# cmgcds/SParSH-AMG

Hardware: AMD Instinct MI355X
Metric: AMG-PCG solve iterations/sec (7-pt 3D Poisson, fp64) + HBM GB/s (roofline: dominant kernel; config.whole_iteration: the iteration) (higher is better)
Workload: dtype f64

## Files before the change

include/sparsh_amg.h:

```cpp
#ifndef SPARSH_AMG_H_
#define SPARSH_AMG_H_

#ifdef __cplusplus
extern "C" {
#endif

#define SPARSH_OK 0
#define SPARSH_EINVAL -1
#define SPARSH_ENODEV -2
#define SPARSH_ESTATE -3
#define SPARSH_ENUMERIC -4
#define SPARSH_ENOCONV -5
#define SPARSH_ECOMM -6

#define SPARSH_AMG 0
#define SPARSH_CG 1
#define SPARSH_PCG 2
#define SPARSH_BICG 3
#define SPARSH_PBICG 4
#define SPARSH_GMRES 5
#define SPARSH_PGMRES 6
#define SPARSH_FCG 7
#define SPARSH_BCG 8
#define SPARSH_MBICG 10
// ... 26 lines not shown
    int extend_until;
    int coarse_factor_mb;
} sparsh_params;

typedef struct sparsh_handle_s *sparsh_handle;

const char *sparsh_last_error(void);
int sparsh_version(void);
int sparsh_device_count(void);
int sparsh_host_cpus(void);

void sparsh_default_params(sparsh_params *p);

int sparsh_create_csr(int nrow, int ncol, const int *rowptr, const int *colindex, const double *val, sparsh_handle *out);
void sparsh_destroy(sparsh_handle h);

int sparsh_setup(sparsh_handle h, const sparsh_params *p);

int sparsh_set_stopping(sparsh_handle h, double tol, int max_iter, int check_every);

int sparsh_set_kernel_config(sparsh_handle h, int kind, int vec, int nt, int remap);

int sparsh_level_format(sparsh_handle h, int level, int *kind, long *stored_entries);

int sparsh_level_layout(sparsh_handle h, int level, long *slots, long *value_blocks, long *meta_bytes);
int sparsh_set_const_slots(sparsh_handle h, int enable);
int sparsh_set_index_compression(sparsh_handle h, int mode);
int sparsh_set_alternate_sweeps(sparsh_handle h, int mode);
int sparsh_set_paired_restriction(sparsh_handle h, int enable);
int sparsh_set_fused_prolongation(sparsh_handle h, int enable);
int sparsh_set_constant_diagonal(sparsh_handle h, int enable);
int sparsh_set_double_sweep(sparsh_handle h, int mode);
int sparsh_set_marching_ops(sparsh_handle h, int mode);
int sparsh_set_zero_start(sparsh_handle h, int enable);
int sparsh_set_deferred_x(sparsh_handle h, int enable);
int sparsh_level_marching_ops(sparsh_handle h, int level, int *on, int *plan, double *table_us, double *marching_us);
int sparsh_set_box_plan(sparsh_handle h, int level, int kernel, int q, int ty, int cz);
int sparsh_set_box_plan_ex(sparsh_handle h, int level, int kernel, int threads, int q, int ty, int cz);
int sparsh_level_box_threads(sparsh_handle h, int level, int *double_threads, int *marching_threads);
int sparsh_debug_box_plan_candidates(int kernel, int nx, int ny, int nz, int part_cap, int cap, int *plans);
int sparsh_level_double_sweep(sparsh_handle h, int level, int *on, int *dims, int *plan, double *single_us, double *double_us);
int sparsh_level_constant_diagonal(sparsh_handle h, int level, int *is_const, double *value);
int sparsh_level_prolong_fused(sparsh_handle h, int level, int *fused);
int sparsh_level_paired(sparsh_handle h, int level, int *paired);
int sparsh_set_fused_zero_sweep(sparsh_handle h, int mode);
int sparsh_set_placement_search(sparsh_handle h, int enable);
int sparsh_placement_info(sparsh_handle h, double *chosen_us, double *worst_us, double *initial_us, int *triples, double *seconds);
int sparsh_set_setup_broadcast(sparsh_handle h, int enable);
int sparsh_setup_share_info(sparsh_handle h, int *built_locally, long *image_bytes);
long sparsh_debug_hierarchy_roundtrip(sparsh_handle h, long truncate_to);
int sparsh_level_index16(sparsh_handle h, int level, long *blocks16, long *blocks);
int sparsh_debug_index16_roundtrip(int nrow, const int *rowptr, const int *colindex, long *blocks16, long *blocks);
int sparsh_set_tile(sparsh_handle h, int enable);
int sparsh_level_tile_rows(sparsh_handle h, int level, int *rows);
int sparsh_bench_comm(sparsh_handle h, int what, int level, int reps, double *avg_seconds);
const char *sparsh_level_kernel(sparsh_handle h, int level);
int sparsh_level_placement(sparsh_handle h, int level, int *nt, int *remap);

int sparsh_setup_host(sparsh_handle h, const sparsh_params *p);

int sparsh_num_levels(sparsh_handle h);
int sparsh_level_info(sparsh_handle h, int level, int *nrow, int *nnz, int *p_ncol, int *p_nnz);
int sparsh_level_csr(sparsh_handle h, int level, int which, int *rowptr, int *colindex, double *val);
int sparsh_coarse_inverse(sparsh_handle h, double *inv);
int sparsh_coarse_info(sparsh_handle h, int *info6, long *bytes);
int sparsh_set_coarse_form(sparsh_handle h, int form, int leaf, int merge_rows);
// ... 233 lines not shown
```

sparsh_amg_amd/__init__.py:

```python
from __future__ import annotations

import ctypes as C
import os

import numpy as np

from . import problems

_HERE = os.path.dirname(os.path.abspath(__file__))
LIB_PATH = os.path.join(_HERE, "libsparsh_amg.so")

SPARSH_AMG, SPARSH_CG, SPARSH_PCG, SPARSH_BICG, SPARSH_PBICG = 0, 1, 2, 3, 4
SPARSH_GMRES, SPARSH_PGMRES = 5, 6
SPARSH_FCG = 7
METHODS = {"amg": SPARSH_AMG, "cg": SPARSH_CG, "pcg": SPARSH_PCG, "bicg": SPARSH_BICG, "pbicg": SPARSH_PBICG,
           "gmres": SPARSH_GMRES, "pgmres": SPARSH_PGMRES}
SPARSH_BCG = 8
BLOCK_METHODS = {"bcg": SPARSH_BCG}
SPARSH_MBICG = 10
UNSYMMETRIC_BLOCK_METHODS = {"mbicg": SPARSH_MBICG}
SPARSH_MBICG_SCALARS, SPARSH_MBICG_PARTIALS = 9, 2048
MBICG_SLOTS = ("ALPHA1", "APR0", "ALPHA", "ASS", "ASAS", "OMEGA1", "BETA", "RR0", "RES")
MBICG_FIN = {"init": 0, "alpha": 1, "omega": 2, "beta_res": 3}
FLEXIBLE_METHODS = {"fcg": SPARSH_FCG}
# ... 63 lines not shown

def _load():
    if not os.path.exists(LIB_PATH):
        raise ImportError(
            f"{LIB_PATH} is missing: build it with `python -c 'import __graft_entry__ as g; g.build()'` "
            "(or `make -C sparsh_amg_amd/csrc`).  There is no pure-Python/CPU fallback."
        )
    L = C.CDLL(LIB_PATH)
    H = C.c_void_p
    P = C.POINTER
    sig = {
        "sparsh_last_error": (C.c_char_p, []),
        "sparsh_version": (C.c_int, []),
        "sparsh_device_count": (C.c_int, []),
        "sparsh_host_cpus": (C.c_int, []),
        "sparsh_default_params": (None, [P(Params)]),
        "sparsh_create_csr": (C.c_int, [C.c_int, C.c_int, c_int_p, c_int_p, c_dbl_p, P(H)]),
        "sparsh_destroy": (None, [H]),
        "sparsh_setup": (C.c_int, [H, P(Params)]),
        "sparsh_setup_host": (C.c_int, [H, P(Params)]),
        "sparsh_set_stopping": (C.c_int, [H, C.c_double, C.c_int, C.c_int]),
        "sparsh_set_kernel_config": (C.c_int, [H, C.c_int, C.c_int, C.c_int, C.c_int]),
        "sparsh_level_placement": (C.c_int, [H, C.c_int, c_int_p, c_int_p]),
        "sparsh_level_format": (C.c_int, [H, C.c_int, c_int_p, C.POINTER(C.c_long)]),
        "sparsh_level_layout": (C.c_int, [H, C.c_int, C.POINTER(C.c_long), C.POINTER(C.c_long), C.POINTER(C.c_long)]),
        "sparsh_set_const_slots": (C.c_int, [H, C.c_int]),
        "sparsh_set_tile": (C.c_int, [H, C.c_int]),
        "sparsh_set_index_compression": (C.c_int, [H, C.c_int]),
        "sparsh_set_alternate_sweeps": (C.c_int, [H, C.c_int]),
        "sparsh_set_paired_restriction": (C.c_int, [H, C.c_int]),
        "sparsh_set_fused_prolongation": (C.c_int, [H, C.c_int]),
        "sparsh_set_constant_diagonal": (C.c_int, [H, C.c_int]),
        "sparsh_set_double_sweep": (C.c_int, [H, C.c_int]),
        "sparsh_set_marching_ops": (C.c_int, [H, C.c_int]),
        "sparsh_set_zero_start": (C.c_int, [H, C.c_int]),
        "sparsh_set_deferred_x": (C.c_int, [H, C.c_int]),
        "sparsh_level_marching_ops": (C.c_int, [H, C.c_int, C.POINTER(C.c_int), C.POINTER(C.c_int), C.POINTER(C.c_double), C.POINTER(C.c_double)]),
        "sparsh_level_double_sweep": (C.c_int, [H, C.c_int, C.POINTER(C.c_int), C.POINTER(C.c_int), C.POINTER(C.c_int), C.POINTER(C.c_double),
                                                  C.POINTER(C.c_double)]),
        "sparsh_level_constant_diagonal": (C.c_int, [H, C.c_int, C.POINTER(C.c_int), C.POINTER(C.c_double)]),
        "sparsh_level_prolong_fused": (C.c_int, [H, C.c_int, C.POINTER(C.c_int)]),
        "sparsh_op_jacobi_prolong": (C.c_int, [H, C.c_int, c_dbl_p, c_dbl_p, c_dbl_p]),
        "sparsh_set_box_plan": (C.c_int, [H, C.c_int, C.c_int, C.c_int, C.c_int, C.c_int]),
        "sparsh_set_box_plan_ex": (C.c_int, [H, C.c_int, C.c_int, C.c_int, C.c_int, C.c_int, C.c_int]),
        "sparsh_level_box_threads": (C.c_int, [H, C.c_int, c_int_p, c_int_p]),
        "sparsh_debug_box_plan_candidates": (C.c_int, [C.c_int, C.c_int, C.c_int, C.c_int, C.c_int, C.c_int, c_int_p]),
        "sparsh_op_spmv_dot": (C.c_int, [H, C.c_int, c_dbl_p, c_dbl_p, c_dbl_p]),
        "sparsh_op_jacobi_dot": (C.c_int, [H, C.c_int, c_dbl_p, c_dbl_p, c_dbl_p, c_dbl_p]),
        "sparsh_level_paired": (C.c_int, [H, C.c_int, C.POINTER(C.c_int)]),
        "sparsh_set_fused_zero_sweep": (C.c_int, [H, C.c_int]),
        "sparsh_set_placement_search": (C.c_int, [H, C.c_int]),
        "sparsh_placement_info": (C.c_int, [H, C.POINTER(C.c_double), C.POINTER(C.c_double), C.POINTER(C.c_double), c_int_p, C.POINTER(C.c_double)]),
        "sparsh_debug_index16_roundtrip": (C.c_int, [C.c_int, c_int_p, c_int_p, C.POINTER(C.c_long), C.POINTER(C.c_long)]),
        "sparsh_set_setup_broadcast": (C.c_int, [H, C.c_int]),
        "sparsh_debug_hierarchy_roundtrip": (C.c_long, [H, C.c_long]),
        "sparsh_setup_share_info": (C.c_int, [H, C.POINTER(C.c_int), C.POINTER(C.c_long)]),
        "sparsh_level_index16": (C.c_int, [H, C.c_int, C.POINTER(C.c_long), C.POINTER(C.c_long)]),
        "sparsh_level_tile_rows": (C.c_int, [H, C.c_int, c_int_p]),
        "sparsh_bench_comm": (C.c_int, [H, C.c_int, C.c_int, C.c_int, c_dbl_p]),
        "sparsh_level_kernel": (C.c_char_p, [H, C.c_int]),
        "sparsh_num_levels": (C.c_int, [H]),
        "sparsh_level_info": (C.c_int, [H, C.c_int, c_int_p, c_int_p, c_int_p, c_int_p]),
        "sparsh_level_csr": (C.c_int, [H, C.c_int, C.c_int, c_int_p, c_int_p, c_dbl_p]),
        "sparsh_coarse_inverse": (C.c_int, [H, c_dbl_p]),
        "sparsh_op_precond_f32": (C.c_int, [H, c_dbl_p, c_dbl_p]),
        "sparsh_level_f32_layout": (C.c_int, [H, C.c_int, c_int_p]),
# ... 354 lines not shown
    def hierarchy_roundtrip(self, truncate_to=-1):
        r = lib.sparsh_debug_hierarchy_roundtrip(self._h, int(truncate_to))
        if r < 0:
            _check(int(r))
        return int(r)

    def setup_share_info(self):
        a, b = C.c_int(), C.c_long()
        _check(lib.sparsh_setup_share_info(self._h, C.byref(a), C.byref(b)))
        return bool(a.value), b.value

    def set_placement_search(self, enable=True):
        _check(lib.sparsh_set_placement_search(self._h, int(bool(enable))))
        return self

    def placement_info(self):
        a, b, c, k, t = C.c_double(), C.c_double(), C.c_double(), C.c_int(), C.c_double()
        _check(lib.sparsh_placement_info(self._h, C.byref(a), C.byref(b), C.byref(c), C.byref(k), C.byref(t)))
        return {"chosen_us": round(a.value, 2), "worst_us": round(b.value, 2), "initial_us": round(c.value, 2), "triples": k.value,
                "seconds": round(t.value, 3)}

    def set_fused_zero_sweep(self, enable=2):
        _check(lib.sparsh_set_fused_zero_sweep(self._h, int(enable)))
        return self

    def set_alternate_sweeps(self, mode=1):
        _check(lib.sparsh_set_alternate_sweeps(self._h, int(mode)))
        return self

    def set_double_sweep(self, mode=1):
        _check(lib.sparsh_set_double_sweep(self._h, int(mode)))
        return self

    def level_double_sweep(self, level):
        on = C.c_int(0)
        dims, plan = (C.c_int * 3)(), (C.c_int * 3)()
        t1, t2 = C.c_double(0.0), C.c_double(0.0)
        _check(lib.sparsh_level_double_sweep(self._h, int(level), C.byref(on), dims, plan, C.byref(t1), C.byref(t2)))
        return {"on": bool(on.value), "grid": list(dims), "points_per_thread": plan[0], "lines_per_tile": plan[1], "planes_per_chunk": plan[2],
                "two_single_sweeps_us": round(t1.value, 2), "double_sweep_us": round(t2.value, 2)}

    def set_deferred_x(self, enable=True):
        _check(lib.sparsh_set_deferred_x(self._h, 1 if enable else 0))
        return self

    def set_zero_start(self, enable=True):
        _check(lib.sparsh_set_zero_start(self._h, 1 if enable else 0))
        return self

    def set_marching_ops(self, mode=1):
        _check(lib.sparsh_set_marching_ops(self._h, int(mode)))
        return self

    def level_marching_ops(self, level):
        on = C.c_int(0)
        plan = (C.c_int * 3)()
        t1, t2 = C.c_double(0.0), C.c_double(0.0)
        _check(lib.sparsh_level_marching_ops(self._h, int(level), C.byref(on), plan, C.byref(t1), C.byref(t2)))
        return {"on": bool(on.value), "points_per_thread": plan[0], "lines_per_tile": plan[1], "planes_per_chunk": plan[2],
                "table_kernel_us": round(t1.value, 2), "marching_kernel_us": round(t2.value, 2)}

    def set_box_plan(self, level, kernel, q=0, ty=0, cz=0, shared_cu=False, threads=1024):
        k = {"double": 2, "marching": 1}.get(kernel, kernel)
        if shared_cu:
            if k != 1:
                raise ValueError("shared_cu is a plan of the marching kernel")
# ... 1209 lines not shown
```

sparsh_amg_amd/csrc/capi.cpp:

```cpp
#include <algorithm>
#include <cmath>
#include <cstdio>
#include <cstdlib>
#include <cstring>
#include <memory>
#include <string>
#include <vector>

#include <hip/hip_runtime_api.h>

#include "../../include/sparsh_amg.h"
#include "bcg_small.hpp"
#include "eig_chol.hpp"
#include "eig_small.hpp"
#include "engine.hpp"

using namespace sparsh;

struct sparsh_handle_s {
    std::unique_ptr<Engine> eng;
    LocalOp cached_op;
    DeepLocal cached_deep;
};

// ... 364 lines not shown
    if (!h || !h->eng) return fail(SPARSH_EINVAL, "null handle");
    if (chosen_us) *chosen_us = h->eng->place_best_us;
    if (worst_us) *worst_us = h->eng->place_worst_us;
    if (initial_us) *initial_us = h->eng->place_first_us;
    if (triples) *triples = h->eng->place_tried;
    if (seconds) *seconds = h->eng->place_seconds;
    return SPARSH_OK;
}

int sparsh_set_fused_zero_sweep(sparsh_handle h, int enable)
{
    if (!h || !h->eng) return fail(SPARSH_EINVAL, "null handle");
    h->eng->kernel_cfg().fuse_cg_zero = enable != 0;
    h->eng->kernel_cfg().cg_nt = enable == 2;
    h->eng->config_changed();
    return SPARSH_OK;
}

int sparsh_set_alternate_sweeps(sparsh_handle h, int enable)
{
    if (!h || !h->eng) return fail(SPARSH_EINVAL, "null handle");
    if (enable < 0 || enable > 2) return fail(SPARSH_EINVAL, "mode must be 0 (never), 1 (where a sweep streams more than the Infinity Cache holds) or 2 (always)");
    h->eng->kernel_cfg().alt_dir = enable;
    h->eng->config_changed();
    return SPARSH_OK;
}

int sparsh_set_double_sweep(sparsh_handle h, int mode)
{
    if (!h || !h->eng) return fail(SPARSH_EINVAL, "null handle");
    if (mode < 0 || mode > 2) return fail(SPARSH_EINVAL, "mode must be 0 (never), 1 (where the setup measures it faster) or 2 (wherever the level is a box grid with a plan)");
    h->eng->kernel_cfg().box2 = mode;
    h->eng->config_changed();
    return SPARSH_OK;
}

int sparsh_level_double_sweep(sparsh_handle h, int level, int *on, int *dims, int *plan, double *single_us, double *double_us)
{
    REQUIRE_READY(h);
    REQUIRE_LEVEL(h, level);
    const DevLevel &L = h->eng->level(level);
    if (on) *on = (!h->eng->distributed() || L.replicated) && box2_applies(L.A, h->eng->kernel_cfg()) ? 1 : 0;
    if (dims) {
        dims[0] = L.A.box_nx;
        dims[1] = L.A.box_ny;
        dims[2] = L.A.box_nz;
    }
    if (plan) {
        plan[0] = L.A.box2.q;
        plan[1] = L.A.box2.ty;
        plan[2] = L.A.box2.cz;
    }
    if (single_us) *single_us = L.box_single_us;
    if (double_us) *double_us = L.box_double_us;
    return SPARSH_OK;
}

int sparsh_set_deferred_x(sparsh_handle h, int enable)
{
    if (!h || !h->eng) return fail(SPARSH_EINVAL, "null handle");
    h->eng->kernel_cfg().defer_x = enable != 0;
    h->eng->config_changed();
    return SPARSH_OK;
}

int sparsh_set_zero_start(sparsh_handle h, int enable)
// ... 2994 lines not shown
```

sparsh_amg_amd/csrc/engine.cpp:

```cpp
#include "engine.hpp"

#include <algorithm>
#include <functional>
#include <cmath>
#include <cstdio>
#include <cstdlib>
#include <cstring>
#include <omp.h>

namespace sparsh {

namespace {
constexpr int kProfEvents = 8192;
}

bool Engine::check(hipError_t e, const char *what)
{
    if (e == hipSuccess) return true;
    error = std::string(what) + ": " + hipGetErrorString(e);
    return false;
}

bool Engine::note_hip(hipError_t e, const char *what)
{
// ... 625 lines not shown
    }
    for (size_t off = 0; good && off < total; off += chunk) {
        const size_t nb = std::min(chunk, total - off);
        if (me == 0) good = check(hipMemcpyAsync(stage, image.data() + off, nb, hipMemcpyHostToDevice, st_), "hipMemcpy");
        good = good && comm_->bcast(stage, nb, 0, st_);
        if (good && me != 0) good = check(hipMemcpyAsync(image.data() + off, stage, nb, hipMemcpyDeviceToHost, st_), "hipMemcpy");
        good = good && check(hipStreamSynchronize(st_), "hipStreamSynchronize");
    }
    if (stage) (void)hipFree(stage);
    if (!good) {
        if (error.empty()) error = "broadcast of the hierarchy failed: " + comm_->error;
        return SPARSH_ECOMM;
    }
    if (me != 0) {
        prm_ = p;
        ready_ = false;
        if (!deserialize_hierarchy(image.data(), image.size(), A0_, H_)) {
            error = H_.error;
            host_ready_ = false;
            return SPARSH_ENUMERIC;
        }
        host_ready_ = true;
        setup_seconds = omp_get_wtime() - t0;
        H_.seconds = setup_seconds;
    }
    return SPARSH_OK;
}

void Engine::tune_box_kernels()
{
    for (size_t l = 0; l + 1 < lev_.size(); ++l) {
        DevLevel &L = lev_[l];
        L.A.box_on = L.A.box1_on = false;
        L.box_single_us = L.box_double_us = L.box1_table_us = L.box1_us = 0.0;
        if (L.A.box2.q <= 0 || (dist_ && !L.replicated) || L.deep || csr_family(L.A, cfg_) != FAM_SDIA_TAB) continue;
        if (cfg_.box2 >= 2) L.A.box_on = true;
        if (cfg_.box1 >= 2) L.A.box1_on = L.A.box1.q > 0;
        const bool time2 = cfg_.box2 == 1, time1 = cfg_.box1 == 1 && L.A.box1.q > 0;
        if (!(time1 || time2)) continue;
        if (L.n < 60000) continue;
        hipEvent_t e0 = nullptr, e1 = nullptr;
        if (hipEventCreate(&e0) != hipSuccess || hipEventCreate(&e1) != hipSuccess) continue;
        CsrArgs a;
        a.b = L.r;
        launch_fill(L.n, 1.0, L.r, st_);
        a.d = L.diag;
        a.omega = prm_.omega;
        auto timed = [&](bool fused) -> double {
            double *p = L.x, *q = L.x2;
            const int launches = fused ? 5 : 10;
            for (int it = 0; it < launches; ++it) {
                if (it == (fused ? 1 : 2)) (void)hipEventRecord(e0, st_);
                if (fused) {
                    launch_box2(L.A, p, a.b, q, prm_.omega, L.fine, st_);
                } else {
                    a.x = p;
                    a.y = q;
                    launch_csr(L.A, OP_JACOBI, a, L.fine, st_, cfg_);
                }
                std::swap(p, q);
            }
            (void)hipEventRecord(e1, st_);
            if (hipEventSynchronize(e1) != hipSuccess) return 1e30;
            float ms = 0.f;
            (void)hipEventElapsedTime(&ms, e0, e1);
            return (double)ms * 1e3 / 4.0;
// ... 2008 lines not shown
```

sparsh_amg_amd/csrc/engine.hpp:

```cpp
#pragma once

#include <memory>
#include <string>
#include <vector>

#include "../../include/sparsh_amg.h"
#include "cheby_bounds.hpp"
#include "coarse.hpp"
#include "comm.hpp"
#include "dist.hpp"
#include "host_setup.hpp"
#include "kernels.hpp"

namespace sparsh {

struct DevLevel {
    bool deep = false;
    int K = 0;
    int npad = 0;
    std::vector<int> layer_end;
    DevDeepPlan dplan[3];
    std::vector<int> blk_first, wblk_first;
    double *xc_stage = nullptr;
    double *b_ext = nullptr;
// ... 116 lines not shown
    static constexpr int kCycleDefaultStride = 3;
    static constexpr long kCycleMaxVisits = 1024;
    void set_cycle(int kind, int stride)
    {
        cycle_kind_ = kind;
        cycle_stride_ = stride;
        config_changed();
    }
    int cycle_kind() const { return cycle_kind_; }
    int cycle_stride() const { return cycle_stride_; }
    bool wk_level(int l) const { return wk_level_for(l, cycle_stride_); }
    long level_visits(int l) const { return level_visits_for(l, cycle_stride_); }
    long cycle_visits() const { return cycle_visits_for(cycle_stride_); }
    int wk_level_count() const;
    size_t wk_bytes() const { return wk_bytes_; }
    void set_nullspace(int kind) { ns_kind_ = kind; }
    int nullspace_built() const { return host_ready_ ? H_.nullspace : SPARSH_NULLSPACE_NONE; }
    bool ns_on() const { return nullspace_built() == SPARSH_NULLSPACE_CONSTANT; }
    int pinned_row() const { return host_ready_ ? H_.pinned_row : -1; }
    double row_defect() const { return host_ready_ ? ns_row_defect_ : 0.0; }
    double col_defect() const { return host_ready_ ? ns_col_defect_ : 0.0; }
    void project(double *v, const double *r = nullptr, double *dot_partial = nullptr, int *dot_nblk = nullptr);
    void project_any(int n, double *v, const double *r, double *part, double *dot_partial, int *dot_nblk);
    int op_project(int n, double *v, const double *r, double *mean, double *dot);
    int cycle_check(int method);
    int cycle_prepare(int method);
    int op_kstep(int l, const double *b, const double *c, const double *d, double *r, double *x, double *scal8);
    int smoother_prepare();
    static constexpr int kSorDefaultSweeps = 6;
    static constexpr long kSorSingleNnz = 0;
    KernelConfig &kernel_cfg() { return cfg_; }
    const KernelConfig &kernel_cfg() const { return cfg_; }
    void config_changed() { drop_graph(); }
    const double *diag_stream(const DevLevel &L) const { return cfg_.const_diag && L.diag_is_const ? nullptr : L.diag; }
    bool zero_start(const DevLevel &L) const { return cfg_.zero_start && (!dist_ || L.replicated) && !L.deep && box2_applies(L.A, cfg_); }
    bool level_prolong_fused(int l) const
    {
        if (l < 1 || l + 1 >= (int)lev_.size() || !cfg_.fuse_prolong || prm_.sweeps < 1 || prm_.precond_fp32) return false;
        const DevLevel &F = lev_[l - 1];
        if (dist_ && !F.replicated) return false;
        return F.P_is_aggregation && !F.deep && (F.pair_aggregates || F.members) && F.R.nrow == lev_[l].n;
    }
    int level_paired(int l) const
    {
        if (!(l + 2 < (int)lev_.size() && prm_.sweeps > 0 && (!dist_ || lev_[l].replicated) && cfg_.pair_restrict)) return 0;
        if (lev_[l].pair_aggregates && resid_pair_applies(lev_[l].A, cfg_)) return 1;
        if (lev_[l].pair_axis != 0 && lev_[l].A.box_nx > 0 && csr_family(lev_[l].A, cfg_) == FAM_SDIA_TAB) return 1 + std::abs(lev_[l].pair_axis);
        return 0;
    }
    double bench_comm(int what, int level, int reps);
    hipStream_t stream() const { return st_; }
    double *partials() const { return part0_; }
    const DevLevel &level(int l) const { return lev_[l]; }
    int n0() const { return A0_.nrow; }
    int local_n0() const { return lev_.empty() ? A0_.nrow : lev_[0].n; }
    void set_comm(std::unique_ptr<Comm> c) { comm_ = std::move(c); }
    void set_overlap(bool on) { overlap_ = on; }
    void set_deep_halo(bool on) { deep_halo_ = on; }
    bool deep_halo() const { return deep_halo_; }
    void set_comm_tuning(int mode) { comm_tune_ = mode; }
    struct CommLevelChoice {
        int rows = 0, halo_rows = 0;
        bool partitioned = false, deep = false;
        double cost_deep_us = 0.0, cost_per_sweep_us = 0.0, cost_replicated_us = 0.0;
    };
    struct CommMeasured {
// ... 397 lines not shown
```

sparsh_amg_amd/csrc/kernels.hip:

```cpp
#include <hip/hip_runtime.h>

#include "kernels.hpp"

#include <algorithm>
#include <type_traits>
#include <vector>

namespace sparsh {

namespace {


__device__ __forceinline__ double wave_sum(double v)
{
#pragma unroll
    for (int off = 32; off > 0; off >>= 1) v += __shfl_down(v, off, 64);
    return v;
}

__device__ __forceinline__ double block_sum(double v, double *red)
{
    v = wave_sum(v);
    const int lane = threadIdx.x & 63, w = threadIdx.x >> 6;
    if (lane == 0) red[w] = v;
    __syncthreads();
    double s = 0.0;
    if (threadIdx.x == 0) {
#pragma unroll
        for (int k = 0; k < kBlock / 64; ++k) s += red[k];
    }
    return s;
}

__device__ __forceinline__ int xcd_remap(int b, int nblk, int mode)
{
// ... 1118 lines not shown

constexpr int kDivWindow = 256;
constexpr unsigned kDivWindowWidth = (unsigned)(2 * kDivWindow + 1) << 20;
struct DivConst {
    double b, r0;
    unsigned fast;
};
__device__ __forceinline__ unsigned div_window_pos(double v)
{
    return ((unsigned)__double2hiint(v) & 0x7fffffffu) - ((unsigned)(1023 - kDivWindow) << 20);
}
__device__ __forceinline__ DivConst make_div_const(double b)
{
    DivConst c;
    c.b = b;
    bool f;
    const double bs0 = __builtin_amdgcn_div_scale(1.0, b, false, &f);
    double r = __builtin_amdgcn_rcp(bs0);
    double e = __builtin_fma(-bs0, r, 1.0);
    r = __builtin_fma(r, e, r);
    e = __builtin_fma(-bs0, r, 1.0);
    r = __builtin_fma(r, e, r);
    c.r0 = r;
    c.fast = div_window_pos(b) < kDivWindowWidth && bs0 == b ? kDivWindowWidth : 0u;
    return c;
}
__device__ __forceinline__ double div_const(double a, const DivConst &c)
{
    if (__builtin_expect(__builtin_amdgcn_ballot_w64(div_window_pos(a) >= c.fast) != 0ull, 0)) return a / c.b;
    const double q0 = a * c.r0;
    const double rem = __builtin_fma(-c.b, q0, a);
    return __builtin_fma(rem, c.r0, q0);
}

struct BoxArgs {
    int nx, ny, nz;
    int TY, CZ, ytiles;
    double c[7];
    double omega;
};

template <int BS, int Q, int TAG, bool ZERO>
__global__ __launch_bounds__(BS) void sdia_box2_kernel(BoxArgs g, const double *__restrict__ x, const double *__restrict__ b,
                                                        double *__restrict__ y)
{
    extern __shared__ double box_lds[];
    const int nx = g.nx, ny = g.ny, nz = g.nz, P = nx * ny, TY = g.TY;
    const int R0 = (TY + 4) * nx;
    const int pitch = nx + 1;
    const int cells = (TY + 4) * pitch + 1;
    double *X0 = box_lds;
    double *X1 = box_lds + cells;
    int wg = blockIdx.x;
    {
        const int nwg = gridDim.x, per = nwg / 8, rem = nwg % 8;
        const int c = wg % 8, r = wg / 8;
        wg = c * per + min(c, rem) + r;
    }
    const int tile = wg % g.ytiles, zc = wg / g.ytiles;
    const int j0 = tile * TY;
    const int z0 = zc * g.CZ, z1 = min(z0 + g.CZ, nz);
    const long base = (long)(j0 - 2) * nx;
    const int tid = threadIdx.x;
    const double c0 = g.c[0], c1 = g.c[1], c2 = g.c[2], c3 = g.c[3], c4 = g.c[4], c5 = g.c[5], c6 = g.c[6], om = g.omega;
    const DivConst dc = make_div_const(c3);
    for (int i = tid; i < 2 * cells; i += BS) box_lds[i] = 0.0;
// ... 87 lines not shown
                    double sum = 0.0;
                    sum = sum + c0 * x1m[q];
                    sum = sum + c1 * X1[s - pitch];
                    sum = sum + c2 * X1[s - 1];
                    sum = sum + c3 * x1c[q];
                    sum = sum + c4 * X1[s + 1];
                    sum = sum + c5 * X1[s + pitch];
                    sum = sum + c6 * x1k[q];
                    const double h = 1.0 * bp[q] + (-1.0) * sum;
                    y[(long)k2 * P + base + p] = x1c[q] + div_const(om * h, dc);
                }
            }
        }
        __syncthreads();
#pragma unroll
        for (int q = 0; q < Q; ++q) {
            if (v1[q]) X1[sidx[q]] = x1k[q];
            x1m[q] = x1c[q];
            x1c[q] = x1k[q];
            xm[q] = xc[q];
            xc[q] = xp[q];
            bp[q] = bk[q];
            if constexpr (ZERO) {
                bk[q] = bq[q];
                bq[q] = xn[q];
                xp[q] = 0.0;
                if (v0[q] && k + 1 <= z1 && k + 2 < nz) xp[q] = div_const(om * xn[q], dc);
            } else {
                xp[q] = xn[q];
                bk[q] = bn[q];
            }
        }
    }
}

enum BoxEpi : int { BOX_SPMV_DOT = 0, BOX_JACOBI_DOT = 1, BOX_RESID_PAIRX = 2, BOX_JACOBI_PROLONG = 3, BOX_JACOBI = 4 };

struct Box1Args {
    const double *x, *b;
    double *y;
    double *y2;
    const double *dc;
    double dconst;
    const int *members;
    int nfine;
    double *partial;
};

template <int BS, int Q, int EPI, int TAG>
__global__ __launch_bounds__(BS) void sdia_box1_kernel(BoxArgs g, Box1Args a)
{
    extern __shared__ double box_lds[];
    __shared__ double red[BS / 64];
    const int nx = g.nx, ny = g.ny, nz = g.nz, P = nx * ny, TY = g.TY;
    const int R0 = (TY + 2) * nx;
    const int pitch = nx + 1;
    const int cells = (TY + 2) * pitch + 1;
    double *X0 = box_lds;
    int wg = blockIdx.x;
    {
        const int nwg = gridDim.x, per = nwg / 8, rem = nwg % 8;
        const int c = wg % 8, r = wg / 8;
        wg = c * per + min(c, rem) + r;
    }
    const int tile = wg % g.ytiles, zc = wg / g.ytiles;
    const int j0 = tile * TY;
// ... 100 lines not shown
                const double rn = lane_from_above(ri, 0.0);
                if (v1[q] && !(tid & 1)) {
                    const long J = row >> 1;
                    double bc = 0.0 + ri;
                    bc = bc + rn;
                    a.y[J] = bc;
                    if (a.y2) a.y2[J] = om * bc / (a.dc ? a.dc[J] : a.dconst);
                }
            }
        }
        __syncthreads();
#pragma unroll
        for (int q = 0; q < Q; ++q) {
            xm[q] = xc[q];
            xc[q] = xp[q];
            xp[q] = xn[q];
            bk[q] = bn[q];
        }
    }
    if constexpr (EPI == BOX_SPMV_DOT || EPI == BOX_JACOBI_DOT) {
        acc = wave_sum(acc);
        const int lane = tid & 63, w = tid >> 6;
        if (lane == 0) red[w] = acc;
        __syncthreads();
        if (tid == 0) {
            double t = 0.0;
#pragma unroll
            for (int q = 0; q < BS / 64; ++q) t += red[q];
            a.partial[blockIdx.x] = t;
        }
    }
}

__device__ __forceinline__ double box_residual(const BoxArgs &g, const double *__restrict__ x, const double *__restrict__ b, int f, int i, int j,
                                               int k)
{
    const int nx = g.nx, P = g.nx * g.ny;
    const double xm2 = k > 0 ? x[f - P] : 0.0;
    const double xm1 = j > 0 ? x[f - nx] : 0.0;
    const double xm0 = i > 0 ? x[f - 1] : 0.0;
    const double xc = x[f];
    const double xp0 = i < nx - 1 ? x[f + 1] : 0.0;
    const double xp1 = j < g.ny - 1 ? x[f + nx] : 0.0;
    const double xp2 = k < g.nz - 1 ? x[f + P] : 0.0;
    const double bi = b[f];
    double sum = 0.0;
    sum = sum + g.c[0] * xm2;
    sum = sum + g.c[1] * xm1;
    sum = sum + g.c[2] * xm0;
    sum = sum + g.c[3] * xc;
    sum = sum + g.c[4] * xp0;
    sum = sum + g.c[5] * xp1;
    sum = sum + g.c[6] * xp2;
    return 1.0 * bi + (-1.0) * sum;
}

template <int AXIS>
__global__ __launch_bounds__(kBlock) void box_resid_pair_kernel(BoxArgs g, int nc, int rev, const double *__restrict__ x, const double *__restrict__ b,
                                                                const double *__restrict__ dc, double dconst, double *__restrict__ bc,
                                                                double *__restrict__ xc)
{
    const int J = blockIdx.x * kBlock + threadIdx.x;
    if (J >= nc) return;
    const int nx = g.nx, ny = g.ny;
    const int cny = AXIS == 1 ? ny / 2 : ny;
    const int i = J % nx, t = J / nx;
// ... 250 lines not shown
}

namespace {

BoxArgs box_args(const DevCsr &A, double omega, const BoxPlan &p = {})
{
    BoxArgs g;
    g.nx = A.box_nx;
    g.ny = A.box_ny;
    g.nz = A.box_nz;
    g.TY = p.ty;
    g.CZ = p.cz;
    g.ytiles = p.ty > 0 ? (g.ny + p.ty - 1) / p.ty : 0;
    for (int u = 0; u < 7; ++u) g.c[u] = A.sd_tab.cval[u];
    g.omega = omega;
    return g;
}

template <class F>
void box_dispatch(const BoxPlan &p, F &&f)
{
    auto with_q = [&](auto bs) {
        if (p.q == 4) f(bs, std::integral_constant<int, 4>{});
        else if (p.q == 3) f(bs, std::integral_constant<int, 3>{});
        else f(bs, std::integral_constant<int, 2>{});
    };
    if (p.threads == 256) with_q(std::integral_constant<int, 256>{});
    else if (p.threads == 512) with_q(std::integral_constant<int, 512>{});
    else with_q(std::integral_constant<int, 1024>{});
}

}

bool box1_applies(const DevCsr &A, const KernelConfig &c)
{
    return c.box1 != 0 && A.box1_on && A.box1.q > 0 && csr_family(A, c) == FAM_SDIA_TAB;
}

int launch_box1(const DevCsr &A, int epi, const CsrArgs &a, bool finest, hipStream_t st)
{
    const BoxArgs g = box_args(A, a.omega, A.box1);
    Box1Args b;
    b.x = a.x;
    b.b = a.b;
    b.y = a.y;
    b.y2 = a.y2;
    b.dc = a.d;
    b.dconst = a.dconst;
    b.members = a.members;
    b.nfine = a.nfine;
    b.partial = a.partial ? a.partial + a.partial_off : nullptr;
    const int nwg = A.box1.workgroups(g.ny, g.nz);
    const dim3 grid(nwg), block(A.box1.threads);
    const size_t lds = box_lds_bytes(1, g.nx, g.TY);
    auto launch = [&](auto e) {
        box_dispatch(A.box1, [&](auto bs, auto q) {
            constexpr int BS = decltype(bs)::value, Q = decltype(q)::value, E = decltype(e)::value;
            if (finest) hipLaunchKernelGGL((sdia_box1_kernel<BS, Q, E, 1>), grid, block, lds, st, g, b);
            else hipLaunchKernelGGL((sdia_box1_kernel<BS, Q, E, 0>), grid, block, lds, st, g, b);
        });
    };
    switch (epi) {
    case BOX_SPMV_DOT: launch(std::integral_constant<int, BOX_SPMV_DOT>{}); break;
    case BOX_JACOBI_DOT: launch(std::integral_constant<int, BOX_JACOBI_DOT>{}); break;
    case BOX_RESID_PAIRX: launch(std::integral_constant<int, BOX_RESID_PAIRX>{}); break;
    case BOX_JACOBI: launch(std::integral_constant<int, BOX_JACOBI>{}); break;
    default: launch(std::integral_constant<int, BOX_JACOBI_PROLONG>{}); break;
    }
    return nwg;
}

bool box2_applies(const DevCsr &A, const KernelConfig &c)
{
    return c.box2 != 0 && A.box_on && A.box2.q > 0 && csr_family(A, c) == FAM_SDIA_TAB;
}

void launch_box2(const DevCsr &A, const double *x, const double *b, double *y, double omega, bool finest, hipStream_t st, bool from_zero)
{
    const BoxArgs g = box_args(A, omega, A.box2);
    const dim3 grid(A.box2.workgroups(g.ny, g.nz)), block(A.box2.threads);
    const size_t lds = box_lds_bytes(2, g.nx, g.TY);
    box_dispatch(A.box2, [&](auto bs, auto q) {
        constexpr int BS = decltype(bs)::value, Q = decltype(q)::value;
        if (from_zero) {
            if (finest) hipLaunchKernelGGL((sdia_box2_kernel<BS, Q, 1, true>), grid, block, lds, st, g, x, b, y);
            else hipLaunchKernelGGL((sdia_box2_kernel<BS, Q, 0, true>), grid, block, lds, st, g, x, b, y);
        } else {
            if (finest) hipLaunchKernelGGL((sdia_box2_kernel<BS, Q, 1, false>), grid, block, lds, st, g, x, b, y);
            else hipLaunchKernelGGL((sdia_box2_kernel<BS, Q, 0, false>), grid, block, lds, st, g, x, b, y);
        }
    });
}

void launch_box_resid_pair(const DevCsr &A, int axis, const double *x, const double *b, const double *dc, double dconst, double omega,
                           double *bc, double *xc, hipStream_t st)
{
    const BoxArgs g = box_args(A, omega);
    const int nc = A.nrow / 2;
    if (nc <= 0) return;
    const dim3 grid((nc + kBlock - 1) / kBlock), block(kBlock);
    const int rev = axis < 0 ? 1 : 0;
    if (axis == 1 || axis == -1)
        hipLaunchKernelGGL(box_resid_pair_kernel<1>, grid, block, 0, st, g, nc, rev, x, b, dc, dconst, bc, xc);
    else
        hipLaunchKernelGGL(box_resid_pair_kernel<2>, grid, block, 0, st, g, nc, rev, x, b, dc, dconst, bc, xc);
}

bool resid_pair_applies(const DevCsr &A, const KernelConfig &c)
{
    return c.pair_restrict && csr_family(A, c) == FAM_SDIA_TAB && sdia_tile_rows(A, c) == 0 && A.nslice > 0;
}

void launch_resid_pair(const DevCsr &A, const CsrArgs &a, bool finest, hipStream_t st, const KernelConfig &c)
{
    bool nt;
    int remap;
// ... 903 lines not shown
```

sparsh_amg_amd/csrc/kernels.hpp:

```cpp
#pragma once

#include <hip/hip_runtime_api.h>

#include <vector>

#include "box_plan.hpp"

namespace sparsh {

struct SdTable {
    int nd = 0;
    int near = 0;
    int off[8] = {0, 0, 0, 0, 0, 0, 0, 0};
    double cval[8] = {0, 0, 0, 0, 0, 0, 0, 0};
};

struct DevCsr {
    int nrow = 0, ncol = 0, nnz = 0;
    int *rowptr = nullptr;
    int *col = nullptr;
    double *val = nullptr;
    int *rowblk = nullptr;
    int nblk = 0;
    unsigned short *col16 = nullptr;
    int *cbase = nullptr;
    int nblk16 = 0;
    int *waveblk = nullptr;
    int nwblk = 0;
    int nslice = 0;
    int *slice_ptr = nullptr;
    int *sell_col = nullptr;
    double *sell_val = nullptr;
    long sell_entries = 0;
    int *sd_ptr = nullptr;
    int *sd_off = nullptr;
    unsigned long long *sd_mask = nullptr;
    double *sd_val = nullptr;
    long sd_slots = 0;
    int *sd_vidx = nullptr;
    double *sd_cval = nullptr;
    long sd_vblocks = 0;
    int *sd_rec = nullptr;
    SdTable sd_tab;
    unsigned long long *sd_tmask = nullptr;
    int *sd_tconf = nullptr;
    bool has_sdia() const { return sd_ptr != nullptr; }
    int box_nx = 0, box_ny = 0, box_nz = 0;
    BoxPlan box2;
    bool box_on = false;
    BoxPlan box1;
    bool box1_on = false;
    int *int_list = nullptr, *bnd_list = nullptr;
    int nint = 0, nbnd = 0;
};

struct KernelConfig {
    int kind = 3;
    int vec = 3;
    bool auto_policy = true;
    bool nt = true;
    int remap = 1;
    bool table = true;
    bool tile = false;
    bool const_slots = true;
    bool place_search = true;
    bool cg_nt = true;
    bool fuse_cg_zero = true;
    int alt_dir = 1;
    bool defer_x = true;
    bool zero_start = true;
    int box1 = 1;
    int box2 = 1;
    bool const_diag = true;
    bool fuse_prolong = true;
    bool pair_restrict = true;
    int idx16 = 1;
};

enum CsrFamily : int { FAM_CSR_BLOCK = 0, FAM_CSR_WAVE = 1, FAM_SELL = 2, FAM_SDIA = 3, FAM_SDIA_TAB = 4, FAM_CSR_ROWLANE = 5, FAM_CSR_ROWLANE16 = 6 };

constexpr int kBlock = 256;
constexpr int kEwGridMax = 2048;
constexpr int kStreamNnz = 2048;
constexpr int kWaveNnz = 512;
constexpr int kSdRecInts = 48;
constexpr int kSdConstBit = 1 << 30;
constexpr int kSdPlainBit = 1 << 29;
constexpr int kSdPtrMask = (1 << 29) - 1;
constexpr int kCsrPad = 4;

enum CsrOp : int {
    OP_SPMV = 0,
    OP_RESID = 1,
    OP_JACOBI = 2,
    OP_ADD = 3,
    OP_SPMV_DOT = 4,
    OP_RESNORM = 5,
    OP_JACOBI_DOT = 6,
    OP_JACOBI_PROLONG = 8,
    OP_CHEBY = 9,
    OP_CHEBY_DOT = 10,
    OP_RESID_PAIR = 7
};

struct CsrArgs {
// ... 281 lines not shown
```

Before: 711.4.

## Add branch-free box stencil kernels using clamped buffer loads and masked stores

```diff
diff --git a/include/sparsh_amg.h b/include/sparsh_amg.h
--- a/include/sparsh_amg.h
+++ b/include/sparsh_amg.h
@@ -82,6 +82,7 @@
 int sparsh_set_constant_diagonal(sparsh_handle h, int enable);
 int sparsh_set_double_sweep(sparsh_handle h, int mode);
 int sparsh_set_marching_ops(sparsh_handle h, int mode);
+int sparsh_set_box_step(sparsh_handle h, int step);
 int sparsh_set_zero_start(sparsh_handle h, int enable);
 int sparsh_set_deferred_x(sparsh_handle h, int enable);
 int sparsh_level_marching_ops(sparsh_handle h, int level, int *on, int *plan, double *table_us, double *marching_us);
diff --git a/sparsh_amg_amd/__init__.py b/sparsh_amg_amd/__init__.py
--- a/sparsh_amg_amd/__init__.py
+++ b/sparsh_amg_amd/__init__.py
@@ -119,6 +119,7 @@
         "sparsh_set_fused_prolongation": (C.c_int, [H, C.c_int]),
         "sparsh_set_constant_diagonal": (C.c_int, [H, C.c_int]),
         "sparsh_set_double_sweep": (C.c_int, [H, C.c_int]),
+        "sparsh_set_box_step": (C.c_int, [H, C.c_int]),
         "sparsh_set_marching_ops": (C.c_int, [H, C.c_int]),
         "sparsh_set_zero_start": (C.c_int, [H, C.c_int]),
         "sparsh_set_deferred_x": (C.c_int, [H, C.c_int]),
@@ -539,6 +540,10 @@
         _check(lib.sparsh_set_double_sweep(self._h, int(mode)))
         return self
 
+    def set_box_step(self, step=1):
+        _check(lib.sparsh_set_box_step(self._h, int(step)))
+        return self
+
     def level_double_sweep(self, level):
         on = C.c_int(0)
         dims, plan = (C.c_int * 3)(), (C.c_int * 3)()
diff --git a/sparsh_amg_amd/csrc/box_step.hpp b/sparsh_amg_amd/csrc/box_step.hpp
--- /dev/null
+++ b/sparsh_amg_amd/csrc/box_step.hpp
@@ -0,0 +1,33 @@
+#pragma once
+
+#if defined(__HIPCC__)
+#define SPARSH_BOX_HD __host__ __device__ inline
+#else
+#define SPARSH_BOX_HD inline
+#endif
+
+namespace sparsh {
+
+SPARSH_BOX_HD int box_step_base(int nx, int P, int line0)
+{
+    const long o = (long)line0 * nx;
+    return o < 0 ? 0 : (o < P ? (int)o : P - 1);
+}
+SPARSH_BOX_HD int box_step_lane(int nx, int P, int line0, int p)
+{
+    const long o = (long)line0 * nx + p;
+    return (o < 0 ? 0 : (o < P ? (int)o : P - 1)) - box_step_base(nx, P, line0);
+}
+
+SPARSH_BOX_HD int box_step_plane(int nz, int k) { return k < 0 ? 0 : (k < nz ? k : nz - 1); }
+
+SPARSH_BOX_HD long box_step_index(int nx, int ny, int nz, int line0, int p, int k)
+{
+    const int P = nx * ny;
+    return (long)box_step_plane(nz, k) * P + box_step_base(nx, P, line0) + box_step_lane(nx, P, line0, p);
+}
+
+SPARSH_BOX_HD int box_step_first(int kernel, int z0) { return kernel == 2 ? z0 - 1 : z0; }
+SPARSH_BOX_HD int box_step_last(int kernel, int z1) { return kernel == 2 ? z1 : z1 - 1; }
+
+}
diff --git a/sparsh_amg_amd/csrc/capi.cpp b/sparsh_amg_amd/csrc/capi.cpp
--- a/sparsh_amg_amd/csrc/capi.cpp
+++ b/sparsh_amg_amd/csrc/capi.cpp
@@ -420,6 +420,14 @@
     if (mode < 0 || mode > 2) return fail(SPARSH_EINVAL, "mode must be 0 (never), 1 (where the setup measures it faster) or 2 (wherever the level is a box grid with a plan)");
     h->eng->kernel_cfg().box2 = mode;
     h->eng->config_changed();
+    return SPARSH_OK;
+}
+
+int sparsh_set_box_step(sparsh_handle h, int step)
+{
+    if (!h || !h->eng) return fail(SPARSH_EINVAL, "null handle");
+    if (step < 0 || step > 1) return fail(SPARSH_EINVAL, "step must be 0 (branches around the points a lane does not own) or 1 (every lane issues every load and store)");
+    h->eng->set_box_step(step);
     return SPARSH_OK;
 }
 
diff --git a/sparsh_amg_amd/csrc/engine.cpp b/sparsh_amg_amd/csrc/engine.cpp
--- a/sparsh_amg_amd/csrc/engine.cpp
+++ b/sparsh_amg_amd/csrc/engine.cpp
@@ -681,6 +681,7 @@
     for (size_t l = 0; l + 1 < lev_.size(); ++l) {
         DevLevel &L = lev_[l];
         L.A.box_on = L.A.box1_on = false;
+        L.A.box_step = cfg_.box_step;
         L.box_single_us = L.box_double_us = L.box1_table_us = L.box1_us = 0.0;
         if (L.A.box2.q <= 0 || (dist_ && !L.replicated) || L.deep || csr_family(L.A, cfg_) != FAM_SDIA_TAB) continue;
         if (cfg_.box2 >= 2) L.A.box_on = true;
diff --git a/sparsh_amg_amd/csrc/engine.hpp b/sparsh_amg_amd/csrc/engine.hpp
--- a/sparsh_amg_amd/csrc/engine.hpp
+++ b/sparsh_amg_amd/csrc/engine.hpp
@@ -172,6 +172,12 @@
     KernelConfig &kernel_cfg() { return cfg_; }
     const KernelConfig &kernel_cfg() const { return cfg_; }
     void config_changed() { drop_graph(); }
+    void set_box_step(int step)
+    {
+        cfg_.box_step = step;
+        for (DevLevel &L : lev_) L.A.box_step = step;
+        config_changed();
+    }
     const double *diag_stream(const DevLevel &L) const { return cfg_.const_diag && L.diag_is_const ? nullptr : L.diag; }
     bool zero_start(const DevLevel &L) const { return cfg_.zero_start && (!dist_ || L.replicated) && !L.deep && box2_applies(L.A, cfg_); }
     bool level_prolong_fused(int l) const
diff --git a/sparsh_amg_amd/csrc/kernels.hip b/sparsh_amg_amd/csrc/kernels.hip
--- a/sparsh_amg_amd/csrc/kernels.hip
+++ b/sparsh_amg_amd/csrc/kernels.hip
@@ -1,6 +1,7 @@
 #include <hip/hip_runtime.h>
 
 #include "kernels.hpp"
+#include "box_step.hpp"
 
 #include <algorithm>
 #include <type_traits>
@@ -1185,6 +1186,19 @@
     const double rem = __builtin_fma(-c.b, q0, a);
     return __builtin_fma(rem, c.r0, q0);
 }
+__device__ __forceinline__ DivConst make_div_const_uniform(double b)
+{
+    DivConst c = make_div_const(b);
+    c.r0 = __hiloint2double(__builtin_amdgcn_readfirstlane(__double2hiint(c.r0)), __builtin_amdgcn_readfirstlane(__double2loint(c.r0)));
+    return c;
+}
+__device__ __forceinline__ double div_const(double a, const DivConst &c, bool on)
+{
+    if (__builtin_expect(__builtin_amdgcn_ballot_w64(on && div_window_pos(a) >= c.fast) != 0ull, 0)) return a / c.b;
+    const double q0 = a * c.r0;
+    const double rem = __builtin_fma(-c.b, q0, a);
+    return __builtin_fma(rem, c.r0, q0);
+}
 
 struct BoxArgs {
     int nx, ny, nz;
@@ -1338,6 +1352,172 @@
             }
         }
     }
+}
+
+constexpr unsigned kBoxRegionBytes = 4u * kBoxBlock * sizeof(double);
+typedef unsigned box_u2 __attribute__((ext_vector_type(2)));
+__device__ __forceinline__ unsigned box_lane_bytes(int lane) { return ((unsigned)lane & (4u * kBoxBlock - 1)) * (unsigned)sizeof(double); }
+__device__ __forceinline__ __amdgpu_buffer_rsrc_t box_region(const double *pl)
+{
+    return __builtin_amdgcn_make_buffer_rsrc(const_cast<double *>(pl), 0, (int)kBoxRegionBytes, 0x00020000);
+}
+__device__ __forceinline__ double box_at(const double *pl, unsigned d8)
+{
+    return __builtin_bit_cast(double, __builtin_amdgcn_raw_buffer_load_b64(box_region(pl), d8, 0, 0));
+}
+__device__ __forceinline__ void box_store(double *pl, unsigned d8, bool on, double v)
+{
+    __builtin_amdgcn_raw_buffer_store_b64(__builtin_bit_cast(box_u2, v), box_region(pl), on ? d8 : kBoxRegionBytes, 0, 0);
+}
+
+template <int BS, int Q, int TAG, bool ZERO>
+__global__ __launch_bounds__(BS) void sdia_box2s_kernel(BoxArgs g, const double *__restrict__ x, const double *__restrict__ b,
+                                                         double *__restrict__ y)
+{
+    extern __shared__ double box_lds[];
+    const int nx = g.nx, ny = g.ny, nz = g.nz, P = nx * ny, TY = g.TY;
+    const int R0 = (TY + 4) * nx;
+    const int pitch = nx + 1;
+    const int cells = (TY + 4) * pitch + 1;
+    double *X0 = box_lds;
+    double *X1 = box_lds + cells;
+    int wg = blockIdx.x;
+    {
+        const int nwg = gridDim.x, per = nwg / 8, rem = nwg % 8;
+        const int c = wg % 8, r = wg / 8;
+        wg = c * per + min(c, rem) + r;
+    }
+    const int tile = wg % g.ytiles, zc = wg / g.ytiles;
+    const int j0 = tile * TY;
+    const int z0 = zc * g.CZ, z1 = min(z0 + g.CZ, nz);
+    const int tid = threadIdx.x;
+    const double c0 = g.c[0], c1 = g.c[1], c2 = g.c[2], c3 = g.c[3], c4 = g.c[4], c5 = g.c[5], c6 = g.c[6], om = g.omega;
+    const DivConst dc = make_div_const_uniform(c3);
+    for (int i = tid; i < 2 * cells; i += BS) box_lds[i] = 0.0;
+    const double *src = ZERO ? b : x;
+    bool v0[Q], v1[Q], v2[Q];
+    int sidx[Q], ridx[Q];
+    unsigned d8[Q];
+    double xm[Q], xc[Q], xp[Q], bk[Q], bp[Q], x1m[Q], x1c[Q];
+    double bq[Q];
+    const int tb = box_step_base(nx, P, j0 - 2);
+    const int ks = box_step_first(2, z0);
+#pragma unroll
+    for (int q = 0; q < Q; ++q) {
+        const int p = tid + BS * q;
+        const int lr = p / nx;
+        const int jr = j0 - 2 + lr;
+        sidx[q] = p + lr + 1;
+        v0[q] = p < R0 && jr >= 0 && jr < ny;
+        v1[q] = v0[q] && lr >= 1 && lr <= TY + 2;
+        v2[q] = v0[q] && lr >= 2 && lr <= TY + 1;
+        ridx[q] = v1[q] ? sidx[q] : pitch + 1;
+        d8[q] = box_lane_bytes(box_step_lane(nx, P, j0 - 2, p));
+        bp[q] = x1m[q] = x1c[q] = bq[q] = 0.0;
+        const double lm = box_at(src + (long)box_step_plane(nz, ks - 1) * P + tb, d8[q]);
+        const double lc = box_at(src + (long)box_step_plane(nz, ks) * P + tb, d8[q]);
+        const double lp = box_at(src + (long)box_step_plane(nz, ks + 1) * P + tb, d8[q]);
+        const bool om_ = v0[q] && ks >= 1, oc = v0[q] && ks >= 0, op = v0[q] && ks + 1 < nz;
+        if constexpr (ZERO) {
+            xm[q] = om_ ? div_const(om * lm, dc, om_) : 0.0;
+            bk[q] = oc ? lc : 0.0;
+            xc[q] = oc ? div_const(om * bk[q], dc, oc) : 0.0;
+            bq[q] = op ? lp : 0.0;
+            xp[q] = op ? div_const(om * bq[q], dc, op) : 0.0;
+        } else {
+            const double lb = box_at(b + (long)box_step_plane(nz, ks) * P + tb, d8[q]);
+            xm[q] = om_ ? lm : 0.0;
+            xc[q] = oc ? lc : 0.0;
+            xp[q] = op ? lp : 0.0;
+            bk[q] = v1[q] && ks >= 0 ? lb : 0.0;
+        }
+    }
+    __syncthreads();
+    auto step = [&](const int k, auto stage2, auto prefetch) {
+        constexpr bool kPrefetch = decltype(prefetch)::value;
+        const bool plane = k >= 0 && k < nz;
+        const bool nextx = k + 2 < nz, nextb = k + 1 < nz;
+        double xn[Q], bn[Q];
+        if constexpr (kPrefetch) {
+            const double *srcn = src + (long)box_step_plane(nz, k + 2) * P + tb;
+            const double *bnext = b + (long)box_step_plane(nz, k + 1) * P + tb;
+#pragma unroll
+            for (int q = 0; q < Q; ++q) {
+                xn[q] = box_at(srcn, d8[q]);
+                if constexpr (!ZERO) bn[q] = box_at(bnext, d8[q]);
+            }
+        }
+#pragma unroll
+        for (int q = 0; q < Q; ++q)
+            if (v0[q]) X0[sidx[q]] = xc[q];
+        __syncthreads();
+        double x1k[Q];
+#pragma unroll
+        for (int q = 0; q < Q; ++q) {
+            const int s = ridx[q];
+            const bool on = plane && v1[q];
+            double sum = 0.0;
+            sum = sum + c0 * xm[q];
+            sum = sum + c1 * X0[s - pitch];
+            sum = sum + c2 * X0[s - 1];
+            sum = sum + c3 * xc[q];
+            sum = sum + c4 * X0[s + 1];
+            sum = sum + c5 * X0[s + pitch];
+            sum = sum + c6 * xp[q];
+            const double h = 1.0 * bk[q] + (-1.0) * sum;
+            const double r = xc[q] + div_const(om * h, dc, on);
+            x1k[q] = on ? r : 0.0;
+        }
+        if constexpr (decltype(stage2)::value) {
+            double *yk = y + (long)(k - 1) * P + tb;
+#pragma unroll
+            for (int q = 0; q < Q; ++q) {
+                const int s = ridx[q];
+                double sum = 0.0;
+                sum = sum + c0 * x1m[q];
+                sum = sum + c1 * X1[s - pitch];
+                sum = sum + c2 * X1[s - 1];
+                sum = sum + c3 * x1c[q];
+                sum = sum + c4 * X1[s + 1];
+                sum = sum + c5 * X1[s + pitch];
+                sum = sum + c6 * x1k[q];
+                const double h = 1.0 * bp[q] + (-1.0) * sum;
+                box_store(yk, d8[q], v2[q], x1c[q] + div_const(om * h, dc, v2[q]));
+            }
+        }
+        __syncthreads();
+#pragma unroll
+        for (int q = 0; q < Q; ++q) {
+            if (v1[q]) X1[sidx[q]] = x1k[q];
+            x1m[q] = x1c[q];
+            x1c[q] = x1k[q];
+            xm[q] = xc[q];
+            xc[q] = xp[q];
+            bp[q] = bk[q];
+            if constexpr (ZERO) bk[q] = bq[q];
+            if constexpr (kPrefetch) {
+                const bool onx = v0[q] && nextx;
+                if constexpr (ZERO) {
+                    bq[q] = onx ? xn[q] : 0.0;
+                    xp[q] = onx ? div_const(om * xn[q], dc, onx) : 0.0;
+                } else {
+                    xp[q] = onx ? xn[q] : 0.0;
+                    bk[q] = v1[q] && nextb ? bn[q] : 0.0;
+                }
+            } else {
+                xp[q] = 0.0;
+                if constexpr (ZERO) bq[q] = 0.0;
+                else bk[q] = 0.0;
+            }
+        }
+    };
+    constexpr std::true_type yes{};
+    constexpr std::false_type no{};
+    step(ks, no, yes);
+    step(ks + 1, no, yes);
+    const int last = box_step_last(2, z1);
+    for (int k = ks + 2; k < last; ++k) step(k, yes, yes);
+    step(last, yes, no);
 }
 
 enum BoxEpi : int { BOX_SPMV_DOT = 0, BOX_JACOBI_DOT = 1, BOX_RESID_PAIRX = 2, BOX_JACOBI_PROLONG = 3, BOX_JACOBI = 4 };
@@ -1504,6 +1684,162 @@
     }
 }
 
+template <int BS, int Q, int EPI, int TAG>
+__global__ __launch_bounds__(BS) void sdia_box1s_kernel(BoxArgs g, Box1Args a)
+{
+    extern __shared__ double box_lds[];
+    __shared__ double red[BS / 64];
+    const int nx = g.nx, ny = g.ny, nz = g.nz, P = nx * ny, TY = g.TY;
+    const int R0 = (TY + 2) * nx;
+    const int pitch = nx + 1;
+    const int cells = (TY + 2) * pitch + 1;
+    double *X0 = box_lds;
+    int wg = blockIdx.x;
+    {
+        const int nwg = gridDim.x, per = nwg / 8, rem = nwg % 8;
+        const int c = wg % 8, r = wg / 8;
+        wg = c * per + min(c, rem) + r;
+    }
+    const int tile = wg % g.ytiles, zc = wg / g.ytiles;
+    const int j0 = tile * TY;
+    const int z0 = zc * g.CZ, z1 = min(z0 + g.CZ, nz);
+    const int tid = threadIdx.x;
+    const double c0 = g.c[0], c1 = g.c[1], c2 = g.c[2], c3 = g.c[3], c4 = g.c[4], c5 = g.c[5], c6 = g.c[6], om = g.omega;
+    constexpr bool kNeedsB = EPI != BOX_SPMV_DOT;
+    constexpr bool kDivides = EPI == BOX_JACOBI_DOT || EPI == BOX_JACOBI_PROLONG || EPI == BOX_JACOBI;
+    DivConst dc3 = {1.0, 1.0, 0u};
+    if constexpr (kDivides) dc3 = make_div_const_uniform(c3);
+    for (int i = tid; i < cells; i += BS) X0[i] = 0.0;
+    bool v0[Q], v1[Q];
+    int sidx[Q], ridx[Q];
+    unsigned d8[Q];
+    double xm[Q], xc[Q], xp[Q], bk[Q];
+    const int tb = box_step_base(nx, P, j0 - 1);
+#pragma unroll
+    for (int q = 0; q < Q; ++q) {
+        const int p = tid + BS * q;
+        const int lr = p / nx;
+        const int jr = j0 - 1 + lr;
+        sidx[q] = p + lr + 1;
+        v0[q] = p < R0 && jr >= 0 && jr < ny;
+        v1[q] = v0[q] && lr >= 1 && lr <= TY;
+        ridx[q] = v1[q] ? sidx[q] : pitch + 1;
+        d8[q] = box_lane_bytes(box_step_lane(nx, P, j0 - 1, p));
+        const double lm = box_at(a.x + (long)box_step_plane(nz, z0 - 1) * P + tb, d8[q]);
+        const double lc = box_at(a.x + (long)z0 * P + tb, d8[q]);
+        const double lp = box_at(a.x + (long)box_step_plane(nz, z0 + 1) * P + tb, d8[q]);
+        xm[q] = v0[q] && z0 >= 1 ? lm : 0.0;
+        xc[q] = v0[q] ? lc : 0.0;
+        xp[q] = v0[q] && z0 + 1 < nz ? lp : 0.0;
+        bk[q] = 0.0;
+        if constexpr (kNeedsB) {
+            const double lb = box_at(a.b + (long)z0 * P + tb, d8[q]);
+            bk[q] = v1[q] ? lb : 0.0;
+        }
+    }
+    __syncthreads();
+    double acc = 0.0;
+    auto step = [&](const int k, auto prefetch) {
+        constexpr bool kPrefetch = decltype(prefetch)::value;
+        const bool nextx = k + 2 < nz;
+        double *yk = a.y + (long)k * P + tb;
+        double xn[Q], bn[Q];
+        if constexpr (kPrefetch) {
+            const double *xnext = a.x + (long)box_step_plane(nz, k + 2) * P + tb;
+            const double *bnext = a.b + (long)(k + 1) * P + tb;
+#pragma unroll
+            for (int q = 0; q < Q; ++q) {
+                xn[q] = box_at(xnext, d8[q]);
+                if constexpr (kNeedsB) bn[q] = box_at(bnext, d8[q]);
+            }
+        }
+#pragma unroll
+        for (int q = 0; q < Q; ++q)
+            if (v0[q]) X0[sidx[q]] = xc[q];
+        __syncthreads();
+#pragma unroll
+        for (int q = 0; q < Q; ++q) {
+            const int s = ridx[q];
+            const long row = (long)k * P + tb + (d8[q] >> 3);
+            double sum = 0.0;
+            sum = sum + c0 * xm[q];
+            sum = sum + c1 * X0[s - pitch];
+            sum = sum + c2 * X0[s - 1];
+            sum = sum + c3 * xc[q];
+            sum = sum + c4 * X0[s + 1];
+            sum = sum + c5 * X0[s + pitch];
+            sum = sum + c6 * xp[q];
+            if constexpr (EPI == BOX_SPMV_DOT) {
+                box_store(yk, d8[q], v1[q], sum);
+                acc = v1[q] ? acc + xc[q] * sum : acc;
+            } else if constexpr (EPI == BOX_JACOBI_DOT || EPI == BOX_JACOBI) {
+                const double h = 1.0 * bk[q] + (-1.0) * sum;
+                const double xnew = xc[q] + div_const(om * h, dc3, v1[q]);
+                box_store(yk, d8[q], v1[q], xnew);
+                if constexpr (EPI == BOX_JACOBI_DOT) acc = v1[q] ? acc + xnew * bk[q] : acc;
+            } else if constexpr (EPI == BOX_JACOBI_PROLONG) {
+                const double h = 1.0 * bk[q] + (-1.0) * sum;
+                const double xnew = xc[q] + div_const(om * h, dc3, v1[q]);
+                if (v1[q]) {
+                    if (a.members) {
+                        const i2v m = *reinterpret_cast<const i2v *>(a.members + 2 * row);
+                        a.y2[m.x] = 1.0 * xnew + a.y2[m.x];
+                        if (m.y >= 0) a.y2[m.y] = 1.0 * xnew + a.y2[m.y];
+                    } else {
+                        const long f = 2 * row;
+                        if (f + 1 < a.nfine) {
+                            d2v *pp = reinterpret_cast<d2v *>(a.y2 + f);
+                            d2v v = *pp;
+                            v.x = 1.0 * xnew + v.x;
+                            v.y = 1.0 * xnew + v.y;
+                            *pp = v;
+                        } else {
+                            a.y2[f] = 1.0 * xnew + a.y2[f];
+                        }
+                    }
+                }
+            } else {
+                const double ri = v1[q] ? 1.0 * bk[q] + (-1.0) * sum : 0.0;
+                const double rn = lane_from_above(ri, 0.0);
+                if (v1[q] && !(tid & 1)) {
+                    const long J = row >> 1;
+                    double bc = 0.0 + ri;
+                    bc = bc + rn;
+                    a.y[J] = bc;
+                    if (a.y2) a.y2[J] = om * bc / (a.dc ? a.dc[J] : a.dconst);
+                }
+            }
+        }
+        __syncthreads();
+#pragma unroll
+        for (int q = 0; q < Q; ++q) {
+            xm[q] = xc[q];
+            xc[q] = xp[q];
+            if constexpr (kPrefetch) {
+                xp[q] = v0[q] && nextx ? xn[q] : 0.0;
+                if constexpr (kNeedsB) bk[q] = v1[q] ? bn[q] : 0.0;
+            } else {
+                xp[q] = bk[q] = 0.0;
+            }
+        }
+    };
+    const int last = box_step_last(1, z1);
+    for (int k = box_step_first(1, z0); k < last; ++k) step(k, std::true_type{});
+    step(last, std::false_type{});
+    if constexpr (EPI == BOX_SPMV_DOT || EPI == BOX_JACOBI_DOT) {
+        acc = wave_sum(acc);
+        const int lane = tid & 63, w = tid >> 6;
+        if (lane == 0) red[w] = acc;
+        __syncthreads();
+        if (tid == 0) {
+            double t = 0.0;
+#pragma unroll
+            for (int q = 0; q < BS / 64; ++q) t += red[q];
+            a.partial[blockIdx.x] = t;
+        }
+    }
+}
+
 __device__ __forceinline__ double box_residual(const BoxArgs &g, const double *__restrict__ x, const double *__restrict__ b, int f, int i, int j,
                                                int k)
 {
@@ -1820,6 +2156,8 @@
 
 }
 
+constexpr bool box_step_kernel(int kernel, int q) { return kernel == 2 ? q <= 3 : q >= 3; }
+
 bool box1_applies(const DevCsr &A, const KernelConfig &c)
 {
     return c.box1 != 0 && A.box1_on && A.box1.q > 0 && csr_family(A, c) == FAM_SDIA_TAB;
@@ -1844,6 +2182,13 @@
     auto launch = [&](auto e) {
         box_dispatch(A.box1, [&](auto bs, auto q) {
             constexpr int BS = decltype(bs)::value, Q = decltype(q)::value, E = decltype(e)::value;
+            if constexpr (box_step_kernel(1, Q)) {
+                if (A.box_step) {
+                    if (finest) hipLaunchKernelGGL((sdia_box1s_kernel<BS, Q, E, 1>), grid, block, lds, st, g, b);
+                    else hipLaunchKernelGGL((sdia_box1s_kernel<BS, Q, E, 0>), grid, block, lds, st, g, b);
+                    return;
+                }
+            }
             if (finest) hipLaunchKernelGGL((sdia_box1_kernel<BS, Q, E, 1>), grid, block, lds, st, g, b);
             else hipLaunchKernelGGL((sdia_box1_kernel<BS, Q, E, 0>), grid, block, lds, st, g, b);
         });
@@ -1870,6 +2215,18 @@
     const size_t lds = box_lds_bytes(2, g.nx, g.TY);
     box_dispatch(A.box2, [&](auto bs, auto q) {
         constexpr int BS = decltype(bs)::value, Q = decltype(q)::value;
+        if constexpr (box_step_kernel(2, Q)) {
+            if (A.box_step) {
+                if (from_zero) {
+                    if (finest) hipLaunchKernelGGL((sdia_box2s_kernel<BS, Q, 1, true>), grid, block, lds, st, g, x, b, y);
+                    else hipLaunchKernelGGL((sdia_box2s_kernel<BS, Q, 0, true>), grid, block, lds, st, g, x, b, y);
+                } else {
+                    if (finest) hipLaunchKernelGGL((sdia_box2s_kernel<BS, Q, 1, false>), grid, block, lds, st, g, x, b, y);
+                    else hipLaunchKernelGGL((sdia_box2s_kernel<BS, Q, 0, false>), grid, block, lds, st, g, x, b, y);
+                }
+                return;
+            }
+        }
         if (from_zero) {
             if (finest) hipLaunchKernelGGL((sdia_box2_kernel<BS, Q, 1, true>), grid, block, lds, st, g, x, b, y);
             else hipLaunchKernelGGL((sdia_box2_kernel<BS, Q, 0, true>), grid, block, lds, st, g, x, b, y);
diff --git a/sparsh_amg_amd/csrc/kernels.hpp b/sparsh_amg_amd/csrc/kernels.hpp
--- a/sparsh_amg_amd/csrc/kernels.hpp
+++ b/sparsh_amg_amd/csrc/kernels.hpp
@@ -50,6 +50,7 @@
     bool box_on = false;
     BoxPlan box1;
     bool box1_on = false;
+    int box_step = 1;
     int *int_list = nullptr, *bnd_list = nullptr;
     int nint = 0, nbnd = 0;
 };
@@ -71,6 +72,7 @@
     bool zero_start = true;
     int box1 = 1;
     int box2 = 1;
+    int box_step = 1;
     bool const_diag = true;
     bool fuse_prolong = true;
     bool pair_restrict = true;
```

Result: no change. 715.6, median of 3 (+0.6%).
